# Consensys/gnark

Hardware: AMD Instinct MI355X
Metric: G1 MSM throughput, BN254, 2^24 scalar-muls on one GPU (Groth16 proofs/s at 2^24 constraints in 'groth16') (higher is better)
Workload: dtype u64 Montgomery limbs in memory; 29/28-bit limbs, v_mad_u64_u32 (32x32+64) in registers

## Files before the change

gnark_amd/csrc/common.hip.h:

```cpp
#pragma once
#include <hip/hip_runtime.h>
#include <stdint.h>
#include <stdio.h>
#include <string.h>

#include <chrono>
#include <condition_variable>
#include <atomic>
#include <map>
#include <mutex>
#include <set>
#include <string>
#include <vector>

#include "../../include/gnark_amd.h"
#include "ec.hip.h"

namespace ga {

#if defined(__HIP_DEVICE_COMPILE__) && !defined(__GFX9__)
#error "libgnark_amd: the kernels assume the 64-lane wavefronts of GFX9 / CDNA (gfx950); a wave32 target would compile and compute wrong transforms and sorts"
#endif
#define GA_REQUIRE_WAVE64() static_assert(true, "64-lane wavefronts: enforced for the whole device pass at the top of common.hip.h")

// ... 294 lines not shown
    ~StageTimer() {
        if (idx >= 0) hipEventRecord(ctx->stages[idx].b, st);
    }
};

struct DeviceGuard {
    explicit DeviceGuard(int dev) { hipSetDevice(dev); }
};

static inline int ilog2_u64(uint64_t x) {
    int l = 0;
    while ((1ull << l) < x) l++;
    return l;
}

template <class C, int G>
int msm_windows_device(Ctx* ctx, const void* d_bases, const void* d_scalars, size_t n, bool scalars_mont, int c,
                       int win_lo, int win_hi, void* h_window_sums, bool combine = false);
template <class C>
int msm_plan(int group, size_t n, int* c, int* nwin);
template <class C>
int msm_plan_table(size_t n, int* c, int* nwin, bool batched = false);

struct MsmPrepared {
    size_t n = 0;
    int c = 0, nwin = 0, win_lo = 0, win_hi = 0;
    int nsets = 0;
    bool table = false;
    uint32_t half = 0, nb = 0, seg = 0;
    uint64_t m = 0, max_tasks = 0;
    uint32_t *vals = nullptr, *task_off = nullptr, *task_start = nullptr, *task_key = nullptr, *task_perm = nullptr;
    uint32_t* task_key_by_id = nullptr;
    uint32_t* task_dest = nullptr;
};

template <class C, int G>
int msm_table_build(Ctx* ctx, const void* d_bases, size_t n, int c, void* d_table);
template <class C, int G>
size_t msm_table_point_bytes();
template <class C, int G>
int msm_table_device(Ctx* ctx, const void* d_table, const void* d_scalars, size_t n, bool scalars_mont, int c, void* h_sum, int win_lo = 0,
                     int win_hi = -1);
template <class C, int G>
int msm_table_device_batch(Ctx* ctx, const void* d_table, const void* const* d_scalars, int batch, size_t n, bool scalars_mont, int c,
                           void* h_sums);
template <class C>
int msm_prepare_table_scalars(Ctx* ctx, const void* d_scalars, size_t n, bool scalars_mont, int c, MsmPrepared* P, int slot = 0,
                              int win_lo = 0, int win_hi = -1);
template <class C, int G>
int msm_table_device_reuse(Ctx* ctx, const void* d_table, const MsmPrepared& P, void* h_sum);
template <class C, int G>
int msm_table_device_reuse_multi(Ctx* ctx, const void* const* tables, int ntab, const MsmPrepared& P, void* h_sums);

struct Domain;
template <class C> int ntt_domain_new(Ctx* ctx, uint64_t n, Domain** out);
template <class C> int ntt_domain_fft(Domain* d, void* d_data, int direction, int decimation, int on_coset);
template <class C> int ntt_domain_compute_h(Domain* d, void* d_a, void* d_b, void* d_c);
template <class C> int ntt_domain_h_chain(Domain* d, void* d_v);
template <class C> int ntt_domain_h_combine(Domain* d, void* d_a, const void* d_b, const void* d_c);
void ntt_domain_delete(Domain* d);
Domain* ntt_domain_take_spare(Ctx* ctx, int curve, uint64_t n);
void ntt_domain_give_spare(Ctx* ctx, Domain* d);
int ntt_domain_curve(const Domain* d);
uint64_t ntt_domain_size(const Domain* d);
Ctx* ntt_domain_ctx(const Domain* d);

// ... 47 lines not shown
```

gnark_amd/csrc/msm.hip.h:

```cpp
#pragma once
#include <cstring>
#include <hipcub/hipcub.hpp>
#include <rocprim/device/device_radix_sort.hpp>

#include <string>

#include "common.hip.h"
#include "field29.hip.h"

namespace ga {

constexpr int GA_ACC29_MINW = 4;
#ifndef GA_ACC29_FP2_MINW
#define GA_ACC29_FP2_MINW 2
#endif
constexpr uint32_t MSM_SIGN = 0x80000000u;
constexpr int MSM_HOT_TASKS = 16;
constexpr uint32_t MSM_VHOT_TASKS = 512;
constexpr uint32_t MSM_VHOT_SPLIT = 64;
constexpr int MSM_GROUP = 32;

typedef rocprim::radix_sort_config<rocprim::default_config, rocprim::default_config,
                                   rocprim::radix_sort_onesweep_config<rocprim::kernel_config<1024, 21>, rocprim::kernel_config<1024, 21>, 11,
                                                                       rocprim::block_radix_rank_algorithm::match>>
// ... 336 lines not shown
        if (h < hb) {
            const uint32_t cnt = start[h + 1] - start[h];
            if (cnt) got[u] = atomicAdd(&cursor[(bin << low) | h], cnt);
        }
    }
#pragma unroll
    for (int u = 0; u < U; u++)
        if (kk[u] != 0xFFFFFFFFu) {
            const uint32_t h = kk[u], at = start[h] + rk[u];
            stage_v[at] = vv[u];
            stage_h[at] = (uint16_t)h;
        }
#pragma unroll
    for (int u = 0; u < PER_T; u++) {
        const uint32_t h = t + (uint32_t)u * 1024u;
        if (h < hb) delta[h] = got[u] - start[h];
    }
    __syncthreads();
    const uint32_t total = hi - lo;
    for (uint32_t p = t; p < total; p += blockDim.x) out_vals[p + delta[stage_h[p]]] = stage_v[p];
}

template <class FrP, int BITS>
int msm_fused_sort(Ctx* ctx, const std::string& sfx, hipStream_t st, const void* d_scalars, size_t n, bool scalars_mont, int c, int nwin,
                   int win_lo, int win_hi, bool table, int batch, uint32_t half, uint32_t nb, uint64_t m, uint16_t* keys, uint32_t* vals,
                   uint32_t* vals2, uint32_t* off, int xcd) {
    constexpr uint32_t BINS = 1u << BITS;
    auto key = [&](const char* k) { return std::string(k) + sfx; };
    const int nwl = win_hi - win_lo;
    const int low = msm_key_low(nb, BITS);
    const uint32_t ncls = ((xcd & 1) && (m >= (1ull << 24) || (xcd & 4))) ? MSM_XCDS : 1;
    const int swz = (xcd & 2) ? 1 : 0;
    uint32_t *ghist, *cursor, *bin_off, *seg_off, *gcount, *kcursor;
    GA_CHECK(ctx->scratch_get(key("msm_p1_hist").c_str(), BINS * MSM_XCDS * 4, (void**)&ghist));
    GA_CHECK(ctx->scratch_get(key("msm_p1_cursor").c_str(), BINS * MSM_XCDS * 4, (void**)&cursor));
    GA_CHECK(ctx->scratch_get(key("msm_p1_bin_off").c_str(), (BINS + 1) * 4, (void**)&bin_off));
    GA_CHECK(ctx->scratch_get(key("msm_p2_seg_off").c_str(), (BINS + 1) * 4, (void**)&seg_off));
    const uint32_t hb = 1u << low;
    const uint64_t nkeys = (((uint64_t)nb >> low) + 1) << low;
    GA_CHECK(ctx->scratch_get(key("msm_p2_count").c_str(), nkeys * 4, (void**)&gcount));
    GA_CHECK(ctx->scratch_get(key("msm_p2_cursor").c_str(), nkeys * 4, (void**)&kcursor));
    auto vec = [&](int b) { return batch == 1 ? (const uint32_t*)d_scalars : reinterpret_cast<const uint32_t* const*>(d_scalars)[b]; };
    {
        StageTimer tm(ctx, "msm_digits_pass1", st);
        const uint32_t tile = msm_p1_tile_scalars(nwl);
        const uint64_t ntiles = (n + tile - 1) / tile;
        uint64_t hist_blocks = (ntiles + MSM_XCDS - 1) / MSM_XCDS * MSM_XCDS;
        if (hist_blocks > 2048) hist_blocks = 2048;
        const uint64_t p1_grid = ctx->tun.msm_p1_grid.load(std::memory_order_relaxed);
        uint64_t p1_blocks = ntiles <= p1_grid ? ntiles : p1_grid;
        if (ncls > 1 && p1_blocks < ntiles) p1_blocks = (p1_blocks + MSM_XCDS - 1) / MSM_XCDS * MSM_XCDS;
        GA_HIP_CHECK(hipMemsetAsync(ghist, 0, BINS * ncls * 4, st));
        for (int b = 0; b < batch; b++)
            hipLaunchKernelGGL((msm_digit_hist_kernel<FrP, BITS>), dim3((unsigned)hist_blocks), dim3(256), 0, st, vec(b), (uint64_t)n,
                               scalars_mont ? 1 : 0, c, nwin, win_lo, win_hi, table ? 1 : 0, (uint32_t)b * half, nb, tile, low, ncls, ghist);
        hipLaunchKernelGGL(msm_p1_scan_kernel<BITS>, dim3(1), dim3(1024), 0, st, (const uint32_t*)ghist, ncls, cursor, bin_off, seg_off);
        for (int b = 0; b < batch; b++)
            hipLaunchKernelGGL((msm_digits_pass1_kernel<FrP, BITS>), dim3((unsigned)p1_blocks), dim3(MSM_P1_THREADS), 0, st, vec(b),
                               (uint64_t)n, scalars_mont ? 1 : 0, c, nwin, win_lo, win_hi, table ? 1 : 0, (uint32_t)b * half, nb, tile, (uint64_t)ntiles, low,
                               ncls, cursor, keys, vals);
        GA_KERNEL_CHECK();
    }
    {
        StageTimer tm(ctx, "msm_sort", st);
        unsigned max_seg = (unsigned)(m / MSM_P2_SEG + BINS);
        if (swz) max_seg = (max_seg + MSM_XCDS - 1) / MSM_XCDS * MSM_XCDS + MSM_XCDS;
        GA_HIP_CHECK(hipMemsetAsync(gcount, 0, nkeys * 4, st));
        hipLaunchKernelGGL(msm_p2_count_kernel<BITS>, dim3(max_seg), dim3(1024), 0, st, (const uint16_t*)keys, (const uint32_t*)seg_off,
                           (const uint32_t*)bin_off, hb, low, swz, gcount);
        GA_KERNEL_CHECK();
        size_t sb = 0;
        void* stmp;
        GA_HIP_CHECK(hipcub::DeviceScan::ExclusiveSum(nullptr, sb, gcount, off, (int)(nb + 1), st));
        GA_CHECK(ctx->scratch_get(key("msm_p2_scan_tmp").c_str(), sb + 256, &stmp));
        GA_HIP_CHECK(hipcub::DeviceScan::ExclusiveSum(stmp, sb, gcount, off, (int)(nb + 1), st));
        GA_HIP_CHECK(hipMemcpyAsync(kcursor, off, ((uint64_t)nb + 1) * 4, hipMemcpyDeviceToDevice, st));
        hipLaunchKernelGGL(msm_p2_scatter_kernel<BITS>, dim3(max_seg), dim3(1024), 0, st, (const uint16_t*)keys, (const uint32_t*)vals,
                           (const uint32_t*)seg_off, (const uint32_t*)bin_off, hb, low, swz, kcursor, vals2);
        GA_KERNEL_CHECK();
    }
    return GA_OK;
}

static __global__ void __launch_bounds__(256) msm_offsets_tasks_kernel(const uint32_t* __restrict__ keys, uint64_t m, uint32_t nb, uint32_t seg,
                                                                       uint32_t* __restrict__ off, uint32_t* __restrict__ ntask) {
    __shared__ uint32_t sh[257];
    const uint32_t b = blockIdx.x * blockDim.x + threadIdx.x;
    auto lower = [&](uint32_t key) {
        uint64_t lo = 0, hi = m;
        while (lo < hi) {
            const uint64_t mid = (lo + hi) >> 1;
            if (keys[mid] < key) lo = mid + 1;
            else hi = mid;
        }
        return (uint32_t)lo;
    };
    if (b <= nb) {
        sh[threadIdx.x] = lower(b);
        off[b] = sh[threadIdx.x];
        if (threadIdx.x == blockDim.x - 1 && b < nb) sh[blockDim.x] = lower(b + 1);
    }
    __syncthreads();
    if (b <= nb) ntask[b] = b < nb ? (sh[threadIdx.x + 1] - sh[threadIdx.x] + seg - 1) / seg : 0;
}

static __global__ void msm_tasks_kernel(const uint32_t* __restrict__ off, uint32_t nb, uint32_t seg, uint32_t* __restrict__ ntask) {
    uint32_t b = blockIdx.x * blockDim.x + threadIdx.x;
    if (b > nb) return;
    uint32_t sz = b < nb ? off[b + 1] - off[b] : 0;
    ntask[b] = (sz + seg - 1) / seg;
}

static __global__ void msm_task_init_kernel(uint32_t* __restrict__ task_qkey, uint32_t* __restrict__ task_id, uint32_t n, uint32_t* __restrict__ long_count) {
    uint32_t i = blockIdx.x * blockDim.x + threadIdx.x;
    if (i < n) {
        task_qkey[i] = 0xFFFFFFFFu;
        task_id[i] = i;
    }
    if (i == 0) *long_count = 0;
}

constexpr uint32_t MSM_LONG_TASKS = 64;
static __global__ void msm_task_list_kernel(const uint32_t* __restrict__ off, const uint32_t* __restrict__ task_off, uint32_t nb,
                                            uint32_t seg, int qshift, uint32_t* __restrict__ task_start, uint32_t* __restrict__ task_key,
                                            uint32_t* __restrict__ task_qkey, uint32_t* __restrict__ task_dest, uint32_t* __restrict__ long_list,
                                            uint32_t* __restrict__ long_count) {
    uint32_t b = blockIdx.x * blockDim.x + threadIdx.x;
    if (b >= nb) return;
    uint32_t t0 = task_off[b], t1 = task_off[b + 1];
    uint32_t start = off[b], end = off[b + 1];
    if (t1 - t0 > MSM_LONG_TASKS) {
        long_list[atomicAdd(long_count, 1u)] = b;
        return;
    }
    for (uint32_t t = t0; t < t1; t++) {
        uint32_t len = end - start < seg ? end - start : seg;
        task_start[t] = start;
        task_dest[t] = (t1 - t0 == 1) ? b : nb + t;
        task_key[t] = seg - len;
        task_qkey[t] = (seg - len) >> qshift;
        start += len;
    }
}

static __global__ void msm_task_list_long_kernel(const uint32_t* __restrict__ off, const uint32_t* __restrict__ task_off, uint32_t nb, uint32_t seg,
                                                 int qshift, uint32_t* __restrict__ task_start, uint32_t* __restrict__ task_key,
                                                 uint32_t* __restrict__ task_qkey, uint32_t* __restrict__ task_dest,
                                                 const uint32_t* __restrict__ long_list, const uint32_t* __restrict__ long_count) {
    const uint32_t nl = *long_count;
    for (uint32_t h = blockIdx.x; h < nl; h += gridDim.x) {
        const uint32_t b = long_list[h];
        const uint32_t t0 = task_off[b], t1 = task_off[b + 1];
        const uint32_t start = off[b], end = off[b + 1];
        for (uint32_t t = t0 + threadIdx.x; t < t1; t += blockDim.x) {
            const uint32_t s0 = start + (t - t0) * seg;
            const uint32_t len = end - s0 < seg ? end - s0 : seg;
            task_start[t] = s0;
            task_dest[t] = nb + t;
            task_key[t] = seg - len;
            task_qkey[t] = (seg - len) >> qshift;
        }
    }
}
// ... 566 lines not shown
                       const uint32_t* __restrict__ vhot_count, XYZZ<F>* __restrict__ vtmp, uint32_t part_stride, uint32_t vtmp_stride) {
    __shared__ LazyPt<F> sh[64];
    __shared__ XYZZ<F> shx[64];
    __shared__ uint32_t bad;
    partial += (uint64_t)blockIdx.y * part_stride;
    vtmp += (uint64_t)blockIdx.y * vtmp_stride;
    const uint32_t items = *vhot_count * MSM_VHOT_SPLIT;
    for (uint32_t id = blockIdx.x; id < items; id += gridDim.x) {
        const uint32_t h = id / MSM_VHOT_SPLIT, part = id % MSM_VHOT_SPLIT;
        const uint32_t b = vhot_list[h];
        const uint32_t t0 = task_off[b], t1 = task_off[b + 1];
        const uint32_t per = (t1 - t0 + MSM_VHOT_SPLIT - 1) / MSM_VHOT_SPLIT;
        const uint32_t lo = t0 + part * per < t1 ? t0 + part * per : t1;
        const uint32_t hi = lo + per < t1 ? lo + per : t1;
        block_sum29<F>(hi - lo, [&](uint32_t i) { return &partial[lo + i]; }, &vtmp[id], sh, shx, &bad);
    }
}
template <class F>
__global__ void __launch_bounds__(64)
msm_vhot_stage2_kernel(const XYZZ<F>* __restrict__ vtmp, const uint32_t* __restrict__ vhot_list, const uint32_t* __restrict__ vhot_count,
                       XYZZ<F>* __restrict__ bsum, uint32_t bsum_stride, uint32_t vtmp_stride) {
    static_assert(MSM_VHOT_SPLIT == 64, "one partial result per lane");
    __shared__ LazyPt<F> sh[64];
    __shared__ XYZZ<F> shx[64];
    __shared__ uint32_t bad;
    vtmp += (uint64_t)blockIdx.y * vtmp_stride;
    bsum += (uint64_t)blockIdx.y * bsum_stride;
    const uint32_t nv = *vhot_count;
    for (uint32_t h = blockIdx.x; h < nv; h += gridDim.x)
        block_sum29<F>(MSM_VHOT_SPLIT, [&](uint32_t i) { return &vtmp[h * MSM_VHOT_SPLIT + i]; }, &bsum[vhot_list[h]], sh, shx, &bad);
}

template <class F>
__global__ void msm_merge_kernel(const XYZZ<F>* __restrict__ partial, const uint32_t* __restrict__ task_off, uint32_t nb,
                                 XYZZ<F>* __restrict__ bsum, uint32_t* __restrict__ hot_list, uint32_t* __restrict__ hot_count,
                                 uint32_t* __restrict__ vhot_list, uint32_t* __restrict__ vhot_count, uint32_t part_stride) {
    uint32_t b = blockIdx.x * blockDim.x + threadIdx.x;
    if (b >= nb) return;
    partial += (uint64_t)blockIdx.y * part_stride;
    bsum += (uint64_t)blockIdx.y * nb;
    uint32_t t0 = task_off[b], t1 = task_off[b + 1];
    uint32_t nt = t1 - t0;
    if (nt == 1) return;
    if (nt > MSM_VHOT_TASKS) {
        if (blockIdx.y == 0) vhot_list[atomicAdd(vhot_count, 1u)] = b;
        return;
    }
    if (nt > MSM_HOT_TASKS) {
        if (blockIdx.y == 0) hot_list[atomicAdd(hot_count, 1u)] = b;
        return;
    }
    XYZZ<F> out = xyzz_inf<F>();
    bool exact = true;
    if constexpr (BaseFieldOf<F>::P::N <= 8) {
        LazyPt<F> acc;
        acc.inf = 1;
        for (uint32_t t = t0; t < t1; t++) lazy_acc<F>(acc, load_pod<XYZZ<F>>(&partial[t]));
        exact = false;
        if (!acc.inf) {
            out.zz = Lazy<F>::to_mem(acc.v.zz);
            exact = is_zero(out.zz);
            out.x = Lazy<F>::to_mem(acc.v.x);
            out.y = Lazy<F>::to_mem(acc.v.y);
            out.zzz = Lazy<F>::to_mem(acc.v.zzz);
        }
    }
    if (exact) {
        out = xyzz_inf<F>();
        for (uint32_t t = t0; t < t1; t++) out = add(out, load_pod<XYZZ<F>>(&partial[t]));
    }
    store_pod(&bsum[b], out);
}

template <class F>
__global__ void __launch_bounds__(64)
msm_bit_partial_kernel(const XYZZ<F>* __restrict__ rsum, const XYZZ<F>* __restrict__ lsum, uint32_t groups_per_win,
                       uint32_t chunk_len, int log_chunk, XYZZ<F>* __restrict__ part) {
    __shared__ LazyPt<F> sh[64];
    __shared__ XYZZ<F> shx[64];
    __shared__ uint32_t bad;
    const uint32_t ch = blockIdx.x, b = blockIdx.y, w = blockIdx.z;
    const uint32_t nbits = gridDim.y, chunks = gridDim.x;
    const uint32_t base = ch * chunk_len;
    const XYZZ<F>* R = rsum + (uint64_t)w * groups_per_win;
    XYZZ<F>* dst = &part[((uint64_t)w * nbits + b) * chunks + ch];
    if (b == nbits - 1) {
        const XYZZ<F>* Lp = lsum + (uint64_t)w * groups_per_win;
        block_sum29<F>(chunk_len, [&](uint32_t i) { return &Lp[base + i]; }, dst, sh, shx, &bad);
    } else if ((int)b >= log_chunk) {
        block_sum29<F>(((base >> b) & 1) ? chunk_len : 0u, [&](uint32_t i) { return &R[base + i]; }, dst, sh, shx, &bad);
    } else {
        block_sum29<F>(chunk_len / 2, [&](uint32_t i) { return &R[base + (((i >> b) << (b + 1)) | (1u << b) | (i & ((1u << b) - 1)))]; }, dst, sh,
                       shx, &bad);
    }
}

template <class F>
__global__ void __launch_bounds__(64)
msm_segment_sum29_kernel(const XYZZ<F>* __restrict__ in, uint32_t seg_len, XYZZ<F>* __restrict__ out) {
    __shared__ LazyPt<F> sh[64];
    __shared__ XYZZ<F> shx[64];
    __shared__ uint32_t bad;
    const uint64_t base = (uint64_t)blockIdx.x * seg_len;
    block_sum29<F>(seg_len, [&](uint32_t i) { return &in[base + i]; }, &out[blockIdx.x], sh, shx, &bad);
}

template <class F>
__global__ void __launch_bounds__(64)
msm_segment_sum_kernel(const XYZZ<F>* __restrict__ in, uint32_t seg_len, XYZZ<F>* __restrict__ out) {
    __shared__ XYZZ<F> sh[64];
    const uint64_t base = (uint64_t)blockIdx.x * seg_len;
    XYZZ<F> acc = xyzz_inf<F>();
    for (uint32_t g = threadIdx.x; g < seg_len; g += 64) acc = add(acc, load_pod<XYZZ<F>>(&in[base + g]));
    acc = wave_tree_sum(acc, sh);
    if (threadIdx.x == 0) store_pod(&out[blockIdx.x], acc);
}


template <class FrP>
int msm_prepare(Ctx* ctx, const void* d_scalars, size_t n, bool scalars_mont, int c, int win_lo, int win_hi, bool table,
                MsmPrepared* P, int slot = 0, int batch = 1) {
    hipStream_t st = ctx->work_stream();
    const std::string sfx = slot ? "#1" : "";
    auto key = [&](const char* k) { return std::string(k) + sfx; };
    const int nwin = FrP::BITS / c + 1;
    if (win_hi < 0) win_hi = nwin;
    if (win_lo < 0 || win_hi > nwin || win_lo >= win_hi || c < 2 || c > 24) {
        set_error("msm: bad window range [%d,%d) of %d (c=%d, table=%d)", win_lo, win_hi, nwin, c, (int)table);
        return GA_ERR_INVALID;
    }
    const int nwl = win_hi - win_lo;
    if (n == 0 || n >= (1ull << 31)) {
        set_error("msm: n=%zu outside [1, 2^31)", n);
        return GA_ERR_INVALID;
    }
    if (batch < 1 || (batch > 1 && !table)) {
        set_error("msm: a batch of scalar vectors needs a precomputed table (batch=%d, table=%d)", batch, (int)table);
// ... 42 lines not shown
    uint16_t* key_parts = nullptr;
    if (fused) {
        GA_CHECK(ctx->scratch_get("msm_keys_level1", m * 2, (void**)&key_parts));
        GA_CHECK(ctx->scratch_get("msm_vals_level1", m * 4, (void**)&vals));
    } else {
        GA_CHECK(ctx->scratch_get(key("msm_keys").c_str(), m * 4, (void**)&keys));
        GA_CHECK(ctx->scratch_get(key("msm_vals").c_str(), m * 4, (void**)&vals));
        GA_CHECK(ctx->scratch_get(key("msm_keys2").c_str(), m * 4, (void**)&keys2));
    }
    if (fused) {
        if (msm_p1_bits(nb64) == 11)
            GA_CHECK((msm_fused_sort<FrP, 11>(ctx, sfx, st, d_scalars, n, scalars_mont, c, nwin, win_lo, win_hi, table, batch, half, nb, m, key_parts, vals, vals2, off, xcd)));
        else
            GA_CHECK((msm_fused_sort<FrP, 12>(ctx, sfx, st, d_scalars, n, scalars_mont, c, nwin, win_lo, win_hi, table, batch, half, nb, m, key_parts, vals, vals2, off, xcd)));
    } else {
        {
            StageTimer tm(ctx, "msm_digits", st);
            for (int b = 0; b < batch; b++) {
                const uint32_t* sc = batch == 1 ? (const uint32_t*)d_scalars : reinterpret_cast<const uint32_t* const*>(d_scalars)[b];
                hipLaunchKernelGGL((msm_digits_kernel<FrP>), dim3((unsigned)((n + 255) / 256)), dim3(256), 0, st, sc, (uint64_t)n,
                                   scalars_mont ? 1 : 0, c, nwin, win_lo, win_hi, table ? 1 : 0, (uint32_t)b * half, (uint32_t)nb64,
                                   keys + (uint64_t)b * nwl * n, vals + (uint64_t)b * nwl * n);
            }
            GA_KERNEL_CHECK();
        }
        StageTimer tm(ctx, "msm_sort", st);
        GA_CHECK(msm_sort_pairs(ctx, key("msm_sort_tmp"), keys, keys2, vals, vals2, (size_t)m, end_bit, st));
    }
    {
        StageTimer tm(ctx, "msm_tasks", st);
        uint32_t *long_list, *long_count;
        GA_CHECK(ctx->scratch_get(key("msm_long").c_str(), (max_tasks / MSM_LONG_TASKS + 2) * 4, (void**)&long_list));
        GA_CHECK(ctx->scratch_get(key("msm_long_count").c_str(), 256, (void**)&long_count));
        int kbits = 1;
        while ((1u << kbits) <= seg) kbits++;
        const bool exact = m >= ctx->tun.msm_task_exact_min.load(std::memory_order_relaxed);
        const int qbits = exact || kbits < 7 ? kbits : 7, qshift = kbits - qbits;
        hipLaunchKernelGGL(msm_task_init_kernel, dim3((unsigned)((max_tasks + 255) / 256)), dim3(256), 0, st, task_qkey, task_id, (uint32_t)max_tasks, long_count);
        if (!fused)
            hipLaunchKernelGGL(msm_offsets_tasks_kernel, dim3((nb + 1 + 255) / 256), dim3(256), 0, st, (const uint32_t*)keys2, m, nb, seg, off, ntask);
        else
            hipLaunchKernelGGL(msm_tasks_kernel, dim3((nb + 1 + 255) / 256), dim3(256), 0, st, (const uint32_t*)off, nb, seg, ntask);
        GA_KERNEL_CHECK();
        size_t tmp_bytes = 0;
        GA_HIP_CHECK(hipcub::DeviceScan::ExclusiveSum(nullptr, tmp_bytes, ntask, task_off, (int)(nb + 1), st));
        GA_CHECK(ctx->scratch_get(key("msm_scan_tmp").c_str(), tmp_bytes + 256, &tmp));
        GA_HIP_CHECK(hipcub::DeviceScan::ExclusiveSum(tmp, tmp_bytes, ntask, task_off, (int)(nb + 1), st));
        hipLaunchKernelGGL(msm_task_list_kernel, dim3((nb + 255) / 256), dim3(256), 0, st, (const uint32_t*)off, (const uint32_t*)task_off,
                           nb, seg, qshift, task_start, task_key, task_qkey, task_dest, long_list, long_count);
        hipLaunchKernelGGL(msm_task_list_long_kernel, dim3(256), dim3(256), 0, st, (const uint32_t*)off, (const uint32_t*)task_off, nb, seg,
                           qshift, task_start, task_key, task_qkey, task_dest, (const uint32_t*)long_list, (const uint32_t*)long_count);
        GA_KERNEL_CHECK();
        size_t tb = 0;
        GA_HIP_CHECK((rocprim::radix_sort_pairs<MsmTaskSort>(nullptr, tb, task_qkey, task_key2, task_id, task_perm, (size_t)max_tasks, 0u, (unsigned)(qbits + 1), st)));
        GA_CHECK(ctx->scratch_get(key("msm_tasksort_tmp").c_str(), tb + 256, &tmp));
        GA_HIP_CHECK((rocprim::radix_sort_pairs<MsmTaskSort>(tmp, tb, task_qkey, task_key2, task_id, task_perm, (size_t)max_tasks, 0u, (unsigned)(qbits + 1), st)));
    }
    P->n = n;
    P->c = c;
    P->nwin = nwin;
    P->win_lo = win_lo;
    P->win_hi = win_hi;
    P->nsets = table ? batch : nwl;
    P->table = table;
    P->half = half;
    P->nb = nb;
    P->seg = seg;
    P->m = m;
    P->max_tasks = max_tasks;
    P->vals = vals2;
    P->task_off = task_off;
    P->task_start = task_start;
    P->task_key = task_key2;
    P->task_key_by_id = task_key;
    P->task_perm = task_perm;
    P->task_dest = task_dest;
    return GA_OK;
}


template <class F>
int msm_accumulate_reduce(Ctx* ctx, const void* d_bases, const MsmPrepared& P, XYZZ<F>* out, int horner_c = 0, const void* const* tables = nullptr,
                          int ntab = 1) {
    const uint32_t nb = P.nb, half = P.half, seg = P.seg;
    if (ntab < 1 || ntab > 4 || (ntab > 1 && (!tables || !P.table || P.nsets != 1 || horner_c != 0))) {
        set_error("msm: a multi-table pass takes 2..4 precomputed tables over one prepared scalar vector (ntab=%d, table=%d, sets=%d)", ntab, (int)P.table, P.nsets);
        return GA_ERR_INVALID;
    }
    const int nsets = ntab > 1 ? ntab : P.nsets;
    const int tuned_group = ctx->tun.msm_group.load(std::memory_order_relaxed);
    uint32_t m_groups = tuned_group ? (uint32_t)tuned_group : (uint32_t)MSM_GROUP;
    const uint64_t min_lanes = 32768;
    while (m_groups > 2 && (uint64_t)half * nsets / m_groups < min_lanes) m_groups >>= 1;
    if (m_groups > half) m_groups = half;
    const uint32_t groups_per_win = half / m_groups;
    const uint32_t total_groups = groups_per_win * nsets;
    uint32_t *hot_list, *hot_count;
    XYZZ<F>*partial, *bsum, *gsum, *gsum2, *wsum;
    GA_CHECK(ctx->scratch_get("msm_hot", ((uint64_t)nb + 2) * 4, (void**)&hot_list));
    GA_CHECK(ctx->scratch_get("msm_hot_count", 256, (void**)&hot_count));
    uint32_t* vhot_list;
    XYZZ<F>* vtmp;
    const uint64_t vhot_cap = P.max_tasks / MSM_VHOT_TASKS + 2;
    GA_CHECK(ctx->scratch_get("msm_vhot", vhot_cap * 4, (void**)&vhot_list));
    GA_CHECK(ctx->scratch_get("msm_vhot_tmp", (uint64_t)ntab * vhot_cap * MSM_VHOT_SPLIT * sizeof(XYZZ<F>), (void**)&vtmp));
    GA_CHECK(ctx->scratch_get("msm_bsum_partial", (uint64_t)ntab * ((uint64_t)nb + P.max_tasks) * sizeof(XYZZ<F>), (void**)&bsum));
    partial = bsum + (uint64_t)ntab * nb;
    const uint32_t part_stride = (uint32_t)P.max_tasks, vtmp_stride = (uint32_t)(vhot_cap * MSM_VHOT_SPLIT);
    GA_CHECK(ctx->scratch_get("msm_gsum", (uint64_t)total_groups * sizeof(XYZZ<F>), (void**)&gsum));
    GA_CHECK(ctx->scratch_get("msm_gsum2", ((uint64_t)total_groups / 1024 + 64) * sizeof(XYZZ<F>), (void**)&gsum2));
    GA_CHECK(ctx->scratch_get("msm_wsum", (uint64_t)nsets * sizeof(XYZZ<F>), (void**)&wsum));
    hipStream_t st = ctx->work_stream();
    GA_HIP_CHECK(hipMemsetAsync(hot_count, 0, 8, st));
    uint32_t h_redo_stack = 0;
    uint32_t* h_redo = ctx->pinned_words();
    if (!h_redo) h_redo = &h_redo_stack;
    *h_redo = 0;
    struct PendingRead {
        hipStream_t st;
        bool pending = false;
        ~PendingRead() {
            if (pending) hipStreamSynchronize(st);
        }
    } redo_read{ctx->work_stream()};
    const uint32_t* acc_table = (const uint32_t*)d_bases;
    {
        uint32_t *redo_list, *redo_count, *redo2_list;
        GA_CHECK(ctx->scratch_get("msm_redo", (uint64_t)ntab * (P.max_tasks + 2) * 4, (void**)&redo_list));
        GA_CHECK(ctx->scratch_get("msm_redo2", (uint64_t)ntab * (P.max_tasks + 2) * 4, (void**)&redo2_list));
        GA_CHECK(ctx->scratch_get("msm_redo_count", 256, (void**)&redo_count));
        GA_HIP_CHECK(hipMemsetAsync(redo_count, 0, 8 * ntab, st));
        StageTimer tm(ctx, "msm_accumulate");
        if (!P.table) {
            uint32_t* hat;
            GA_CHECK(ctx->scratch_get("msm_hat_bases", (uint64_t)P.n * sizeof(Affine<F>) + 256, (void**)&hat));
            hipLaunchKernelGGL((msm_hat_bases_kernel<F>), dim3((unsigned)((P.n + 255) / 256)), dim3(256), 0, st, (const Affine<F>*)d_bases,
                               (uint64_t)P.n, hat);
            acc_table = hat;
        }
        constexpr unsigned AT = Table29<F>::THREADS;
        const dim3 grid((unsigned)((P.max_tasks + AT - 1) / AT), (unsigned)ntab);
        MsmTables mt;
        mt.k = (uint32_t)ntab;
        mt.nb = nb;
        mt.max_tasks = (uint32_t)P.max_tasks;
        for (int i = 0; i < 4; i++) mt.t[i] = ntab > 1 ? (const uint32_t*)tables[i < ntab ? i : 0] : acc_table;
        if (ntab == 1 && P.table && !ctx->tun.msm_exact_redo && ctx->is_degenerate(d_bases))
            hipLaunchKernelGGL((msm_accumulate29_kernel<F, true>), grid, dim3(AT), 0, st, mt, (const uint32_t*)P.vals,
                               (const uint32_t*)P.task_start, (const uint32_t*)P.task_key, (const uint32_t*)P.task_key_by_id, (const uint32_t*)P.task_perm, (uint32_t)P.max_tasks, seg,
                               (const uint32_t*)P.task_dest, bsum, redo2_list, redo_count + 1);
        else
            hipLaunchKernelGGL((msm_accumulate29_kernel<F, false>), grid, dim3(AT), 0, st, mt, (const uint32_t*)P.vals,
                               (const uint32_t*)P.task_start, (const uint32_t*)P.task_key, (const uint32_t*)P.task_key_by_id, (const uint32_t*)P.task_perm, (uint32_t)P.max_tasks, seg,
                               (const uint32_t*)P.task_dest, bsum, redo_list, redo_count);
        if (!ctx->tun.msm_exact_redo)
            hipLaunchKernelGGL((msm_accumulate29_retry_kernel<F>), dim3(2048, (unsigned)ntab), dim3(AT), 0, st, mt, (const uint32_t*)P.vals,
                               (const uint32_t*)P.task_start, (const uint32_t*)P.task_key_by_id, seg, (const uint32_t*)redo_list,
                               (const uint32_t*)redo_count, (const uint32_t*)P.task_dest, bsum, redo2_list, redo_count + 1);
        else
            hipLaunchKernelGGL((msm_accumulate29_redo_kernel<F>), dim3(1024, (unsigned)ntab), dim3(64), 0, st, mt, (const uint32_t*)P.vals,
                               (const uint32_t*)P.task_start, (const uint32_t*)P.task_key_by_id, seg, (const uint32_t*)redo_list,
                               (const uint32_t*)redo_count, (const uint32_t*)P.task_dest, bsum);
        hipLaunchKernelGGL((msm_accumulate29_redo_kernel<F>), dim3(1024, (unsigned)ntab), dim3(64), 0, st, mt, (const uint32_t*)P.vals,
                           (const uint32_t*)P.task_start, (const uint32_t*)P.task_key_by_id, seg, (const uint32_t*)redo2_list,
                           (const uint32_t*)(redo_count + 1), (const uint32_t*)P.task_dest, bsum);
        GA_KERNEL_CHECK();
        GA_HIP_CHECK(hipMemcpyAsync(h_redo, redo_count, h_redo == &h_redo_stack ? 4 : 8 * (size_t)ntab, hipMemcpyDeviceToHost, st));
        redo_read.pending = true;
    }
    auto note_degenerate = [&]() {
        if (!P.table) return;
        if (ntab == 1) {
            if ((uint64_t)*h_redo * 4 > P.max_tasks) ctx->mark_degenerate(d_bases);
        } else if (h_redo != &h_redo_stack) {
            for (int i = 0; i < ntab; i++)
                if ((uint64_t)h_redo[2 * i] * 4 > P.max_tasks) ctx->mark_degenerate(tables[i]);
        }
    };
    {
        StageTimer tm(ctx, "msm_merge");
        const unsigned ny = (unsigned)ntab;
        hipLaunchKernelGGL((msm_merge_kernel<F>), dim3((nb + 255) / 256, ny), dim3(256), 0, st, (const XYZZ<F>*)partial,
                           (const uint32_t*)P.task_off, nb, bsum, hot_list, hot_count, vhot_list, hot_count + 1, part_stride);
        hipLaunchKernelGGL((msm_hot_kernel<F>), dim3(512, ny), dim3(64), 0, st, (const XYZZ<F>*)partial, (const uint32_t*)P.task_off,
                           (const uint32_t*)hot_list, (const uint32_t*)hot_count, bsum, nb, part_stride);
        hipLaunchKernelGGL((msm_vhot_stage1_kernel<F>), dim3(2048, ny), dim3(64), 0, st, (const XYZZ<F>*)partial, (const uint32_t*)P.task_off,
                           (const uint32_t*)vhot_list, (const uint32_t*)(hot_count + 1), vtmp, part_stride, vtmp_stride);
        hipLaunchKernelGGL((msm_vhot_stage2_kernel<F>), dim3(256, ny), dim3(64), 0, st, (const XYZZ<F>*)vtmp, (const uint32_t*)vhot_list,
                           (const uint32_t*)(hot_count + 1), bsum, nb, vtmp_stride);
        GA_KERNEL_CHECK();
    }
    const bool big_set = (uint64_t)half * nsets >= ctx->tun.reduce_lazy_min;
    const bool dense_set = P.m >= 16ull * (uint64_t)half * (uint64_t)P.nsets && !(P.table && ctx->is_sparse_set(d_bases));
    const bool lazy_reduce = big_set || dense_set;
    if (!lazy_reduce) {
        StageTimer tm(ctx, "msm_reduce");
        hipLaunchKernelGGL((msm_reduce_groups_kernel<F>), dim3((total_groups + 63) / 64), dim3(64), 0, st, (const XYZZ<F>*)bsum,
                           half, m_groups, groups_per_win, total_groups, gsum);
        const uint32_t sg = 1024;
        if (groups_per_win > 2 * sg) {
            const uint32_t nseg = groups_per_win / sg;
            hipLaunchKernelGGL((msm_segment_sum_kernel<F>), dim3(nseg * nsets), dim3(64), 0, st, (const XYZZ<F>*)gsum, sg, gsum2);
            hipLaunchKernelGGL((msm_segment_sum_kernel<F>), dim3(nsets), dim3(64), 0, st, (const XYZZ<F>*)gsum2, nseg, wsum);
        } else {
            hipLaunchKernelGGL((msm_segment_sum_kernel<F>), dim3(nsets), dim3(64), 0, st, (const XYZZ<F>*)gsum, groups_per_win, wsum);
        }
        GA_KERNEL_CHECK();
        if (horner_c > 0) {
            std::vector<XYZZ<F>> ws((size_t)nsets);
            GA_HIP_CHECK(hipMemcpyAsync(ws.data(), wsum, (size_t)nsets * sizeof(XYZZ<F>), hipMemcpyDeviceToHost, st));
            GA_HIP_CHECK(hipStreamSynchronize(st));
            note_degenerate();
            XYZZ<F> acc = xyzz_inf<F>();
            for (int w = nsets - 1; w >= 0; w--) {
                for (int k = 0; k < horner_c; k++) acc = dbl(acc);
                acc = add(acc, ws[(size_t)w]);
            }
            out[0] = acc;
            return GA_OK;
        }
        GA_HIP_CHECK(hipMemcpyAsync(out, wsum, (size_t)nsets * sizeof(XYZZ<F>), hipMemcpyDeviceToHost, st));
        GA_HIP_CHECK(hipStreamSynchronize(st));
        note_degenerate();
        return GA_OK;
    }
    int nbits = 0;
    while ((1u << nbits) < groups_per_win) nbits++;
    uint32_t sg = 1024;
    while (sg > 64 && (uint64_t)(groups_per_win / sg) * (uint64_t)(nbits + 1) * (uint64_t)nsets < 2048) sg >>= 1;
    const uint32_t chunk_len = groups_per_win > sg ? sg : groups_per_win;
    const uint32_t chunks = groups_per_win / chunk_len;
    int log_chunk = 0;
    while ((1u << log_chunk) < chunk_len) log_chunk++;
    XYZZ<F>*rsum = nullptr, *bpart = nullptr, *bits = nullptr;
    uint32_t *rg_list, *rg_count;
    GA_CHECK(ctx->scratch_get("msm_rsum", (uint64_t)total_groups * sizeof(XYZZ<F>), (void**)&rsum));
    GA_CHECK(ctx->scratch_get("msm_bpart", ((uint64_t)nsets * (nbits + 1) * chunks + 64) * sizeof(XYZZ<F>), (void**)&bpart));
    GA_CHECK(ctx->scratch_get("msm_bits", ((uint64_t)nsets * (nbits + 1) + 64) * sizeof(XYZZ<F>), (void**)&bits));
    GA_CHECK(ctx->scratch_get("msm_redo_groups", ((uint64_t)total_groups + 2) * 4, (void**)&rg_list));
    GA_CHECK(ctx->scratch_get("msm_redo_groups_count", 256, (void**)&rg_count));
    GA_HIP_CHECK(hipMemsetAsync(rg_count, 0, 4, st));
    {
        StageTimer tm(ctx, "msm_reduce");
        hipLaunchKernelGGL((msm_reduce_groups29_kernel<F>), dim3((total_groups + 63) / 64), dim3(64), 0, st, (const XYZZ<F>*)bsum,
                           half, m_groups, groups_per_win, total_groups, gsum, rsum, rg_list, rg_count);
        hipLaunchKernelGGL((msm_reduce_groups_redo_kernel<F>), dim3(256), dim3(64), 0, st, (const XYZZ<F>*)bsum, half, m_groups,
                           groups_per_win, (const uint32_t*)rg_list, (const uint32_t*)rg_count, gsum, rsum);
        hipLaunchKernelGGL((msm_bit_partial_kernel<F>), dim3(chunks, (unsigned)nbits + 1, (unsigned)nsets), dim3(64), 0, st,
                           (const XYZZ<F>*)rsum, (const XYZZ<F>*)gsum, groups_per_win, chunk_len, log_chunk, bpart);
        hipLaunchKernelGGL((msm_segment_sum29_kernel<F>), dim3((unsigned)(nsets * (nbits + 1))), dim3(64), 0, st, (const XYZZ<F>*)bpart,
                           chunks, bits);
        GA_KERNEL_CHECK();
    }
    const int rows = nbits + 1;
    std::vector<XYZZ<F>> hb((size_t)nsets * rows);
    uint32_t h_redo_groups = 0;
    GA_HIP_CHECK(hipMemcpyAsync(hb.data(), bits, (size_t)nsets * rows * sizeof(XYZZ<F>), hipMemcpyDeviceToHost, st));
    GA_HIP_CHECK(hipMemcpyAsync(&h_redo_groups, rg_count, 4, hipMemcpyDeviceToHost, st));
    GA_HIP_CHECK(hipStreamSynchronize(st));
    note_degenerate();
    if (P.table && !big_set) ctx->note_sparse_set(d_bases, (uint64_t)h_redo_groups * 4 > total_groups);
    int log_m = 0;
    while ((1u << log_m) < m_groups) log_m++;
    if (horner_c > 0) {
        const int top = horner_c * (nsets - 1) + log_m + nbits - 1;
        std::vector<std::vector<const XYZZ<F>*>> at((size_t)top + 1);
        for (int w = 0; w < nsets; w++) {
            at[(size_t)(horner_c * w)].push_back(&hb[(size_t)w * rows + nbits]);
            for (int b = 0; b < nbits; b++) at[(size_t)(horner_c * w + log_m + b)].push_back(&hb[(size_t)w * rows + b]);
        }
        XYZZ<F> acc = xyzz_inf<F>();
        for (int pos = top; pos >= 0; pos--) {
            if (pos != top) acc = dbl(acc);
            for (const XYZZ<F>* t : at[(size_t)pos]) acc = add(acc, *t);
        }
        out[0] = acc;
        return GA_OK;
    }
    for (int w = 0; w < nsets; w++) {
        XYZZ<F> acc = xyzz_inf<F>();
        for (int b = nbits - 1; b >= 0; b--) acc = add(dbl(acc), hb[(size_t)w * rows + b]);
        for (int k = 0; k < log_m; k++) acc = dbl(acc);
        out[w] = add(hb[(size_t)w * rows + nbits], acc);
    }
// ... 85 lines not shown
```

Measured before the change: 893.6.

## Compact merge work into a bucket list and coalesce counter memsets

```diff
diff --git a/gnark_amd/csrc/common.hip.h b/gnark_amd/csrc/common.hip.h
--- a/gnark_amd/csrc/common.hip.h
+++ b/gnark_amd/csrc/common.hip.h
@@ -350,6 +350,7 @@
     uint32_t *vals = nullptr, *task_off = nullptr, *task_start = nullptr, *task_key = nullptr, *task_perm = nullptr;
     uint32_t* task_key_by_id = nullptr;
     uint32_t* task_dest = nullptr;
+    uint32_t *merge_list = nullptr, *merge_count = nullptr;
 };
 
 template <class C, int G>
diff --git a/gnark_amd/csrc/msm.hip.h b/gnark_amd/csrc/msm.hip.h
--- a/gnark_amd/csrc/msm.hip.h
+++ b/gnark_amd/csrc/msm.hip.h
@@ -392,13 +392,13 @@
     const uint32_t ncls = ((xcd & 1) && (m >= (1ull << 24) || (xcd & 4))) ? MSM_XCDS : 1;
     const int swz = (xcd & 2) ? 1 : 0;
     uint32_t *ghist, *cursor, *bin_off, *seg_off, *gcount, *kcursor;
-    GA_CHECK(ctx->scratch_get(key("msm_p1_hist").c_str(), BINS * MSM_XCDS * 4, (void**)&ghist));
     GA_CHECK(ctx->scratch_get(key("msm_p1_cursor").c_str(), BINS * MSM_XCDS * 4, (void**)&cursor));
     GA_CHECK(ctx->scratch_get(key("msm_p1_bin_off").c_str(), (BINS + 1) * 4, (void**)&bin_off));
     GA_CHECK(ctx->scratch_get(key("msm_p2_seg_off").c_str(), (BINS + 1) * 4, (void**)&seg_off));
     const uint32_t hb = 1u << low;
     const uint64_t nkeys = (((uint64_t)nb >> low) + 1) << low;
-    GA_CHECK(ctx->scratch_get(key("msm_p2_count").c_str(), nkeys * 4, (void**)&gcount));
+    GA_CHECK(ctx->scratch_get(key("msm_p2_count").c_str(), (nkeys + BINS * MSM_XCDS) * 4, (void**)&gcount));
+    ghist = gcount + nkeys;
     GA_CHECK(ctx->scratch_get(key("msm_p2_cursor").c_str(), nkeys * 4, (void**)&kcursor));
     auto vec = [&](int b) { return batch == 1 ? (const uint32_t*)d_scalars : reinterpret_cast<const uint32_t* const*>(d_scalars)[b]; };
     {
@@ -410,7 +410,7 @@
         const uint64_t p1_grid = ctx->tun.msm_p1_grid.load(std::memory_order_relaxed);
         uint64_t p1_blocks = ntiles <= p1_grid ? ntiles : p1_grid;
         if (ncls > 1 && p1_blocks < ntiles) p1_blocks = (p1_blocks + MSM_XCDS - 1) / MSM_XCDS * MSM_XCDS;
-        GA_HIP_CHECK(hipMemsetAsync(ghist, 0, BINS * ncls * 4, st));
+        GA_HIP_CHECK(hipMemsetAsync(gcount, 0, (nkeys + BINS * ncls) * 4, st));
         for (int b = 0; b < batch; b++)
             hipLaunchKernelGGL((msm_digit_hist_kernel<FrP, BITS>), dim3((unsigned)hist_blocks), dim3(256), 0, st, vec(b), (uint64_t)n,
                                scalars_mont ? 1 : 0, c, nwin, win_lo, win_hi, table ? 1 : 0, (uint32_t)b * half, nb, tile, low, ncls, ghist);
@@ -425,7 +425,6 @@
         StageTimer tm(ctx, "msm_sort", st);
         unsigned max_seg = (unsigned)(m / MSM_P2_SEG + BINS);
         if (swz) max_seg = (max_seg + MSM_XCDS - 1) / MSM_XCDS * MSM_XCDS + MSM_XCDS;
-        GA_HIP_CHECK(hipMemsetAsync(gcount, 0, nkeys * 4, st));
         hipLaunchKernelGGL(msm_p2_count_kernel<BITS>, dim3(max_seg), dim3(1024), 0, st, (const uint16_t*)keys, (const uint32_t*)seg_off,
                            (const uint32_t*)bin_off, hb, low, swz, gcount);
         GA_KERNEL_CHECK();
@@ -477,18 +476,19 @@
         task_qkey[i] = 0xFFFFFFFFu;
         task_id[i] = i;
     }
-    if (i == 0) *long_count = 0;
+    if (i == 0) long_count[0] = long_count[1] = 0;
 }
 
 constexpr uint32_t MSM_LONG_TASKS = 64;
 static __global__ void msm_task_list_kernel(const uint32_t* __restrict__ off, const uint32_t* __restrict__ task_off, uint32_t nb,
                                             uint32_t seg, int qshift, uint32_t* __restrict__ task_start, uint32_t* __restrict__ task_key,
                                             uint32_t* __restrict__ task_qkey, uint32_t* __restrict__ task_dest, uint32_t* __restrict__ long_list,
-                                            uint32_t* __restrict__ long_count) {
+                                            uint32_t* __restrict__ long_count, uint32_t* __restrict__ merge_list) {
     uint32_t b = blockIdx.x * blockDim.x + threadIdx.x;
     if (b >= nb) return;
     uint32_t t0 = task_off[b], t1 = task_off[b + 1];
     uint32_t start = off[b], end = off[b + 1];
+    if (t1 - t0 != 1) merge_list[atomicAdd(long_count + 1, 1u)] = b;
     if (t1 - t0 > MSM_LONG_TASKS) {
         long_list[atomicAdd(long_count, 1u)] = b;
         return;
@@ -1121,44 +1121,45 @@
 }
 
 template <class F>
-__global__ void msm_merge_kernel(const XYZZ<F>* __restrict__ partial, const uint32_t* __restrict__ task_off, uint32_t nb,
+__global__ void __launch_bounds__(256) msm_merge_kernel(const XYZZ<F>* __restrict__ partial, const uint32_t* __restrict__ task_off, uint32_t nb,
+                                 const uint32_t* __restrict__ merge_list, const uint32_t* __restrict__ merge_count,
                                  XYZZ<F>* __restrict__ bsum, uint32_t* __restrict__ hot_list, uint32_t* __restrict__ hot_count,
                                  uint32_t* __restrict__ vhot_list, uint32_t* __restrict__ vhot_count, uint32_t part_stride) {
-    uint32_t b = blockIdx.x * blockDim.x + threadIdx.x;
-    if (b >= nb) return;
     partial += (uint64_t)blockIdx.y * part_stride;
     bsum += (uint64_t)blockIdx.y * nb;
-    uint32_t t0 = task_off[b], t1 = task_off[b + 1];
-    uint32_t nt = t1 - t0;
-    if (nt == 1) return;
-    if (nt > MSM_VHOT_TASKS) {
-        if (blockIdx.y == 0) vhot_list[atomicAdd(vhot_count, 1u)] = b;
-        return;
-    }
-    if (nt > MSM_HOT_TASKS) {
-        if (blockIdx.y == 0) hot_list[atomicAdd(hot_count, 1u)] = b;
-        return;
-    }
-    XYZZ<F> out = xyzz_inf<F>();
-    bool exact = true;
-    if constexpr (BaseFieldOf<F>::P::N <= 8) {
-        LazyPt<F> acc;
-        acc.inf = 1;
-        for (uint32_t t = t0; t < t1; t++) lazy_acc<F>(acc, load_pod<XYZZ<F>>(&partial[t]));
-        exact = false;
-        if (!acc.inf) {
-            out.zz = Lazy<F>::to_mem(acc.v.zz);
-            exact = is_zero(out.zz);
-            out.x = Lazy<F>::to_mem(acc.v.x);
-            out.y = Lazy<F>::to_mem(acc.v.y);
-            out.zzz = Lazy<F>::to_mem(acc.v.zzz);
-        }
-    }
-    if (exact) {
-        out = xyzz_inf<F>();
-        for (uint32_t t = t0; t < t1; t++) out = add(out, load_pod<XYZZ<F>>(&partial[t]));
-    }
-    store_pod(&bsum[b], out);
+    const uint32_t nm = *merge_count;
+    for (uint32_t q = blockIdx.x * blockDim.x + threadIdx.x; q < nm; q += gridDim.x * blockDim.x) {
+        const uint32_t b = merge_list[q];
+        uint32_t t0 = task_off[b], t1 = task_off[b + 1];
+        uint32_t nt = t1 - t0;
+        if (nt > MSM_VHOT_TASKS) {
+            if (blockIdx.y == 0) vhot_list[atomicAdd(vhot_count, 1u)] = b;
+            continue;
+        }
+        if (nt > MSM_HOT_TASKS) {
+            if (blockIdx.y == 0) hot_list[atomicAdd(hot_count, 1u)] = b;
+            continue;
+        }
+        XYZZ<F> out = xyzz_inf<F>();
+        if constexpr (BaseFieldOf<F>::P::N <= 8) {
+            LazyPt<F> acc;
+            acc.inf = 1;
+            for (uint32_t t = t0; t < t1; t++) lazy_acc<F>(acc, load_pod<XYZZ<F>>(&partial[t]));
+            if (!acc.inf) {
+                out.zz = Lazy<F>::to_mem(acc.v.zz);
+                if (is_zero(out.zz)) {
+                    hot_list[atomicAdd(hot_count, 1u)] = b;
+                    continue;
+                }
+                out.x = Lazy<F>::to_mem(acc.v.x);
+                out.y = Lazy<F>::to_mem(acc.v.y);
+                out.zzz = Lazy<F>::to_mem(acc.v.zzz);
+            }
+        } else {
+            for (uint32_t t = t0; t < t1; t++) out = add(out, load_pod<XYZZ<F>>(&partial[t]));
+        }
+        store_pod(&bsum[b], out);
+    }
 }
 
 template <class F>
@@ -1300,6 +1301,8 @@
         uint32_t *long_list, *long_count;
         GA_CHECK(ctx->scratch_get(key("msm_long").c_str(), (max_tasks / MSM_LONG_TASKS + 2) * 4, (void**)&long_list));
         GA_CHECK(ctx->scratch_get(key("msm_long_count").c_str(), 256, (void**)&long_count));
+        GA_CHECK(ctx->scratch_get(key("msm_merge_list").c_str(), ((uint64_t)nb + 2) * 4, (void**)&P->merge_list));
+        P->merge_count = long_count + 1;
         int kbits = 1;
         while ((1u << kbits) <= seg) kbits++;
         const bool exact = m >= ctx->tun.msm_task_exact_min.load(std::memory_order_relaxed);
@@ -1315,7 +1318,7 @@
         GA_CHECK(ctx->scratch_get(key("msm_scan_tmp").c_str(), tmp_bytes + 256, &tmp));
         GA_HIP_CHECK(hipcub::DeviceScan::ExclusiveSum(tmp, tmp_bytes, ntask, task_off, (int)(nb + 1), st));
         hipLaunchKernelGGL(msm_task_list_kernel, dim3((nb + 255) / 256), dim3(256), 0, st, (const uint32_t*)off, (const uint32_t*)task_off,
-                           nb, seg, qshift, task_start, task_key, task_qkey, task_dest, long_list, long_count);
+                           nb, seg, qshift, task_start, task_key, task_qkey, task_dest, long_list, long_count, P->merge_list);
         hipLaunchKernelGGL(msm_task_list_long_kernel, dim3(256), dim3(256), 0, st, (const uint32_t*)off, (const uint32_t*)task_off, nb, seg,
                            qshift, task_start, task_key, task_qkey, task_dest, (const uint32_t*)long_list, (const uint32_t*)long_count);
         GA_KERNEL_CHECK();
@@ -1365,8 +1368,8 @@
     const uint32_t total_groups = groups_per_win * nsets;
     uint32_t *hot_list, *hot_count;
     XYZZ<F>*partial, *bsum, *gsum, *gsum2, *wsum;
-    GA_CHECK(ctx->scratch_get("msm_hot", ((uint64_t)nb + 2) * 4, (void**)&hot_list));
-    GA_CHECK(ctx->scratch_get("msm_hot_count", 256, (void**)&hot_count));
+    GA_CHECK(ctx->scratch_get("msm_hot", ((uint64_t)ntab * nb + 2) * 4, (void**)&hot_list));
+    GA_CHECK(ctx->scratch_get("msm_counters", 256, (void**)&hot_count));
     uint32_t* vhot_list;
     XYZZ<F>* vtmp;
     const uint64_t vhot_cap = P.max_tasks / MSM_VHOT_TASKS + 2;
@@ -1379,7 +1382,7 @@
     GA_CHECK(ctx->scratch_get("msm_gsum2", ((uint64_t)total_groups / 1024 + 64) * sizeof(XYZZ<F>), (void**)&gsum2));
     GA_CHECK(ctx->scratch_get("msm_wsum", (uint64_t)nsets * sizeof(XYZZ<F>), (void**)&wsum));
     hipStream_t st = ctx->work_stream();
-    GA_HIP_CHECK(hipMemsetAsync(hot_count, 0, 8, st));
+    GA_HIP_CHECK(hipMemsetAsync(hot_count, 0, 64, st));
     uint32_t h_redo_stack = 0;
     uint32_t* h_redo = ctx->pinned_words();
     if (!h_redo) h_redo = &h_redo_stack;
@@ -1396,8 +1399,7 @@
         uint32_t *redo_list, *redo_count, *redo2_list;
         GA_CHECK(ctx->scratch_get("msm_redo", (uint64_t)ntab * (P.max_tasks + 2) * 4, (void**)&redo_list));
         GA_CHECK(ctx->scratch_get("msm_redo2", (uint64_t)ntab * (P.max_tasks + 2) * 4, (void**)&redo2_list));
-        GA_CHECK(ctx->scratch_get("msm_redo_count", 256, (void**)&redo_count));
-        GA_HIP_CHECK(hipMemsetAsync(redo_count, 0, 8 * ntab, st));
+        redo_count = hot_count + 8;
         StageTimer tm(ctx, "msm_accumulate");
         if (!P.table) {
             uint32_t* hat;
@@ -1448,8 +1450,10 @@
     {
         StageTimer tm(ctx, "msm_merge");
         const unsigned ny = (unsigned)ntab;
-        hipLaunchKernelGGL((msm_merge_kernel<F>), dim3((nb + 255) / 256, ny), dim3(256), 0, st, (const XYZZ<F>*)partial,
-                           (const uint32_t*)P.task_off, nb, bsum, hot_list, hot_count, vhot_list, hot_count + 1, part_stride);
+        const unsigned merge_blocks = (nb + 255) / 256 < 1024 ? (nb + 255) / 256 : 1024;
+        hipLaunchKernelGGL((msm_merge_kernel<F>), dim3(merge_blocks, ny), dim3(256), 0, st, (const XYZZ<F>*)partial,
+                           (const uint32_t*)P.task_off, nb, (const uint32_t*)P.merge_list, (const uint32_t*)P.merge_count, bsum, hot_list,
+                           hot_count, vhot_list, hot_count + 1, part_stride);
         hipLaunchKernelGGL((msm_hot_kernel<F>), dim3(512, ny), dim3(64), 0, st, (const XYZZ<F>*)partial, (const uint32_t*)P.task_off,
                            (const uint32_t*)hot_list, (const uint32_t*)hot_count, bsum, nb, part_stride);
         hipLaunchKernelGGL((msm_vhot_stage1_kernel<F>), dim3(2048, ny), dim3(64), 0, st, (const XYZZ<F>*)partial, (const uint32_t*)P.task_off,
@@ -1506,8 +1510,7 @@
     GA_CHECK(ctx->scratch_get("msm_bpart", ((uint64_t)nsets * (nbits + 1) * chunks + 64) * sizeof(XYZZ<F>), (void**)&bpart));
     GA_CHECK(ctx->scratch_get("msm_bits", ((uint64_t)nsets * (nbits + 1) + 64) * sizeof(XYZZ<F>), (void**)&bits));
     GA_CHECK(ctx->scratch_get("msm_redo_groups", ((uint64_t)total_groups + 2) * 4, (void**)&rg_list));
-    GA_CHECK(ctx->scratch_get("msm_redo_groups_count", 256, (void**)&rg_count));
-    GA_HIP_CHECK(hipMemsetAsync(rg_count, 0, 4, st));
+    rg_count = hot_count + 2;
     {
         StageTimer tm(ctx, "msm_reduce");
         hipLaunchKernelGGL((msm_reduce_groups29_kernel<F>), dim3((total_groups + 63) / 64), dim3(64), 0, st, (const XYZZ<F>*)bsum,
```

After: 891.4 (median of 2 runs). No clear change (-0.2%).

## Replace per-bit chunked bucket partial sums with row/column decomposition

Applied to the files above, without the earlier changes.

```diff
diff --git a/gnark_amd/csrc/msm.hip.h b/gnark_amd/csrc/msm.hip.h
--- a/gnark_amd/csrc/msm.hip.h
+++ b/gnark_amd/csrc/msm.hip.h
@@ -1163,35 +1163,40 @@
 
 template <class F>
 __global__ void __launch_bounds__(64)
-msm_bit_partial_kernel(const XYZZ<F>* __restrict__ rsum, const XYZZ<F>* __restrict__ lsum, uint32_t groups_per_win,
-                       uint32_t chunk_len, int log_chunk, XYZZ<F>* __restrict__ part) {
+msm_rowcol_sum_kernel(const XYZZ<F>* __restrict__ rsum, const XYZZ<F>* __restrict__ lsum, uint32_t groups_per_win, int lo_bits,
+                      XYZZ<F>* __restrict__ rc) {
     __shared__ LazyPt<F> sh[64];
     __shared__ XYZZ<F> shx[64];
     __shared__ uint32_t bad;
-    const uint32_t ch = blockIdx.x, b = blockIdx.y, w = blockIdx.z;
-    const uint32_t nbits = gridDim.y, chunks = gridDim.x;
-    const uint32_t base = ch * chunk_len;
-    const XYZZ<F>* R = rsum + (uint64_t)w * groups_per_win;
-    XYZZ<F>* dst = &part[((uint64_t)w * nbits + b) * chunks + ch];
-    if (b == nbits - 1) {
-        const XYZZ<F>* Lp = lsum + (uint64_t)w * groups_per_win;
-        block_sum29<F>(chunk_len, [&](uint32_t i) { return &Lp[base + i]; }, dst, sh, shx, &bad);
-    } else if ((int)b >= log_chunk) {
-        block_sum29<F>(((base >> b) & 1) ? chunk_len : 0u, [&](uint32_t i) { return &R[base + i]; }, dst, sh, shx, &bad);
-    } else {
-        block_sum29<F>(chunk_len / 2, [&](uint32_t i) { return &R[base + (((i >> b) << (b + 1)) | (1u << b) | (i & ((1u << b) - 1)))]; }, dst, sh,
-                       shx, &bad);
-    }
-}
-
+    const uint32_t nlo = 1u << lo_bits, nhi = groups_per_win >> lo_bits;
+    const uint32_t x = blockIdx.x, kind = blockIdx.y, w = blockIdx.z;
+    if (x >= (kind == 1 ? nlo : nhi)) return;
+    const XYZZ<F>* R = (kind == 2 ? lsum : rsum) + (uint64_t)w * groups_per_win;
+    XYZZ<F>* out = rc + (uint64_t)w * (2 * nhi + nlo);
+    if (kind == 1) block_sum29<F>(nhi, [&](uint32_t i) { return &R[(uint64_t)i * nlo + x]; }, &out[nhi + x], sh, shx, &bad);
+    else block_sum29<F>(nlo, [&](uint32_t i) { return &R[(uint64_t)x * nlo + i]; }, &out[kind == 0 ? x : nhi + nlo + x], sh, shx, &bad);
+}
 template <class F>
 __global__ void __launch_bounds__(64)
-msm_segment_sum29_kernel(const XYZZ<F>* __restrict__ in, uint32_t seg_len, XYZZ<F>* __restrict__ out) {
+msm_bit_rows_kernel(const XYZZ<F>* __restrict__ rc, int lo_bits, int hi_bits, XYZZ<F>* __restrict__ bits) {
     __shared__ LazyPt<F> sh[64];
     __shared__ XYZZ<F> shx[64];
     __shared__ uint32_t bad;
-    const uint64_t base = (uint64_t)blockIdx.x * seg_len;
-    block_sum29<F>(seg_len, [&](uint32_t i) { return &in[base + i]; }, &out[blockIdx.x], sh, shx, &bad);
+    const uint32_t nlo = 1u << lo_bits, nhi = 1u << hi_bits;
+    const uint32_t b = blockIdx.x, nbits = gridDim.x - 1, w = blockIdx.y;
+    const XYZZ<F>* row = rc + (uint64_t)w * (2 * nhi + nlo);
+    const XYZZ<F>* col = row + nhi;
+    const XYZZ<F>* lrow = col + nlo;
+    XYZZ<F>* dst = &bits[(uint64_t)w * (nbits + 1) + b];
+    auto with_bit = [](uint32_t i, uint32_t k) { return ((i >> k) << (k + 1)) | (1u << k) | (i & ((1u << k) - 1)); };
+    if (b == nbits) {
+        block_sum29<F>(nhi, [&](uint32_t i) { return &lrow[i]; }, dst, sh, shx, &bad);
+    } else if (b < (uint32_t)lo_bits) {
+        block_sum29<F>(nlo / 2, [&](uint32_t i) { return &col[with_bit(i, b)]; }, dst, sh, shx, &bad);
+    } else {
+        const uint32_t k = b - (uint32_t)lo_bits;
+        block_sum29<F>(nhi / 2, [&](uint32_t i) { return &row[with_bit(i, k)]; }, dst, sh, shx, &bad);
+    }
 }
 
 template <class F>
@@ -1494,16 +1499,12 @@
     }
     int nbits = 0;
     while ((1u << nbits) < groups_per_win) nbits++;
-    uint32_t sg = 1024;
-    while (sg > 64 && (uint64_t)(groups_per_win / sg) * (uint64_t)(nbits + 1) * (uint64_t)nsets < 2048) sg >>= 1;
-    const uint32_t chunk_len = groups_per_win > sg ? sg : groups_per_win;
-    const uint32_t chunks = groups_per_win / chunk_len;
-    int log_chunk = 0;
-    while ((1u << log_chunk) < chunk_len) log_chunk++;
+    const int lo_bits = nbits / 2, hi_bits = nbits - lo_bits;
+    const uint32_t nlo = 1u << lo_bits, nhi = 1u << hi_bits;
     XYZZ<F>*rsum = nullptr, *bpart = nullptr, *bits = nullptr;
     uint32_t *rg_list, *rg_count;
     GA_CHECK(ctx->scratch_get("msm_rsum", (uint64_t)total_groups * sizeof(XYZZ<F>), (void**)&rsum));
-    GA_CHECK(ctx->scratch_get("msm_bpart", ((uint64_t)nsets * (nbits + 1) * chunks + 64) * sizeof(XYZZ<F>), (void**)&bpart));
+    GA_CHECK(ctx->scratch_get("msm_bpart", ((uint64_t)nsets * (2 * nhi + nlo) + 64) * sizeof(XYZZ<F>), (void**)&bpart));
     GA_CHECK(ctx->scratch_get("msm_bits", ((uint64_t)nsets * (nbits + 1) + 64) * sizeof(XYZZ<F>), (void**)&bits));
     GA_CHECK(ctx->scratch_get("msm_redo_groups", ((uint64_t)total_groups + 2) * 4, (void**)&rg_list));
     GA_CHECK(ctx->scratch_get("msm_redo_groups_count", 256, (void**)&rg_count));
@@ -1514,10 +1515,10 @@
                            half, m_groups, groups_per_win, total_groups, gsum, rsum, rg_list, rg_count);
         hipLaunchKernelGGL((msm_reduce_groups_redo_kernel<F>), dim3(256), dim3(64), 0, st, (const XYZZ<F>*)bsum, half, m_groups,
                            groups_per_win, (const uint32_t*)rg_list, (const uint32_t*)rg_count, gsum, rsum);
-        hipLaunchKernelGGL((msm_bit_partial_kernel<F>), dim3(chunks, (unsigned)nbits + 1, (unsigned)nsets), dim3(64), 0, st,
-                           (const XYZZ<F>*)rsum, (const XYZZ<F>*)gsum, groups_per_win, chunk_len, log_chunk, bpart);
-        hipLaunchKernelGGL((msm_segment_sum29_kernel<F>), dim3((unsigned)(nsets * (nbits + 1))), dim3(64), 0, st, (const XYZZ<F>*)bpart,
-                           chunks, bits);
+        hipLaunchKernelGGL((msm_rowcol_sum_kernel<F>), dim3(nhi, 3, (unsigned)nsets), dim3(64), 0, st, (const XYZZ<F>*)rsum,
+                           (const XYZZ<F>*)gsum, groups_per_win, lo_bits, bpart);
+        hipLaunchKernelGGL((msm_bit_rows_kernel<F>), dim3((unsigned)nbits + 1, (unsigned)nsets), dim3(64), 0, st, (const XYZZ<F>*)bpart,
+                           lo_bits, hi_bits, bits);
         GA_KERNEL_CHECK();
     }
     const int rows = nbits + 1;
```

New measurement: 906.8 before, 911.5 after (median of 4 runs). No clear change (+0.5%).
